# megapose6d/megapose6d

Hardware: NVIDIA H100
Metric: pose hypotheses/sec through render+coarse+5x refine (higher is better)
Workload: dtype f16

## Files before the change

include/mpx.h:

```cpp
#ifndef MPX_H_
#define MPX_H_

#include <stddef.h>
#include <stdint.h>

#ifdef __cplusplus
extern "C" {
#endif

#define MPX_ABI_VERSION 5

int mpx_abi_version(void);
int mpx_act_dtype(void);
const char* mpx_last_error(void);
long long mpx_launch_count(void);
int mpx_set_sm_limit(int n_sms);
int mpx_sm_count(void);
int mpx_profile_enable(int on);
int mpx_profile_summary(double* conv_ms, double* conv_flops, long long* conv_launches);

typedef struct mpx_meshdb mpx_meshdb;
int mpx_meshdb_create(int n_meshes, const float* h_verts, const float* h_normals,
                      const float* h_colors, const int64_t* h_vert_offsets, const int32_t* h_faces,
                      const int64_t* h_face_offsets, mpx_meshdb** out);
// ... 37 lines not shown
                          int c_in, void* d_x, int c_pad, int ch_per_view, const float* d_depth_norm_z,
                          void* d_workspace, size_t workspace_bytes, void* stream);

int mpx_pose_init_autodepth(const float* d_points, int n_pts, const int32_t* d_label_idx,
                            const float* d_bboxes, const float* d_K, const float* d_R, int n,
                            float* d_TCO, void* stream);

int mpx_normalize_T(const float* d_T_in, int n, float* d_T_out, void* stream);

int mpx_crop_geometry(const float* d_points, int n_pts, const int32_t* d_label_idx,
                      const float* d_TCO, const float* d_K, const float* d_tCR, int n, float lamb,
                      int im_h, int im_w, int out_h, int out_w, float* d_boxes_rend,
                      float* d_boxes_crop, float* d_K_crop, void* stream);

int mpx_multiview_cameras(const float* d_TCO, const float* d_tCR, int n, const float* h_offsets,
                          int n_extra, float* d_TCV_O, void* stream);

int mpx_pose_update(const float* d_TCO, const float* d_K_crop, const float* d_pose9,
                    const float* d_tCR, int n, float* d_TCO_out, void* stream);

int mpx_topk_per_group(const float* d_logits, int n_groups, int m, int k, int32_t* d_idx,
                       void* stream);

int mpx_image_to_nhwc4(const float* d_images_nchw, int b, int c, int h, int w, float* d_out_nhwc4,
                       void* stream);
int mpx_roi_align(const float* d_img_nhwc4, int b, int h, int w, const int32_t* d_im_idx,
                  const float* d_boxes, int n, int c, int out_h, int out_w, float* d_out,
                  void* stream);
int mpx_roi_align_fused(const float* d_img_nhwc4, int b, int h, int w, const int32_t* d_im_idx,
                        const float* d_boxes, int n, int c, int out_h, int out_w, void* d_x,
                        int c_pad, const float* d_depth_norm_z, int depth_norm_kind, void* stream);

size_t mpx_net_input_bytes(int n, int h, int w, int c_pad);

int mpx_conv2d(const void* d_x, int n, int h, int w, int c_in, const void* d_w,
                    const float* d_bias, int c_out, int r, int s, int stride, int pad_lo_h,
                    int pad_lo_w, int pad_hi_h, int pad_hi_w, int relu, const void* d_residual,
                    void* d_out, int block_n, int max_ctas, void* stream);

int mpx_conv2d_splitk(const void* d_x, int n, int h, int w, int c_in, const void* d_w,
                           const float* d_bias, int c_out, int r, int s, int stride, int pad_lo_h,
                           int pad_lo_w, int pad_hi_h, int pad_hi_w, int relu, const void* d_residual,
                           void* d_out, int block_n, int splits, void* stream);

#define MPX_CONV_NET_SPLITK 8
#define MPX_CONV_NO_PDL 512
#define MPX_CONV_SPLITK_CAP2 262144
#define MPX_CONV_SPLITK_CAP1 524288
#define MPX_CONV_NEVER_C64 4194304
#define MPX_CONV_FORCE_IM2COL 8388608
#define MPX_CONV_FORCE_C64 67108864
#define MPX_CONV_NEVER_PP 134217728
#define MPX_CONV_FORCE_PP 268435456
int mpx_conv_set_mode(int mode);

int mpx_maxpool3x3s2(const void* d_x, int n, int h, int w, int c, void* d_out, void* stream);

int mpx_avgpool_linear(const void* d_x, int n, int hw, int c, const float* d_w, const float* d_b,
                       int out_dim, float* d_out, void* stream);

typedef struct mpx_net mpx_net;
int mpx_net_create(int c_pad, int out_dim, const void* const* h_conv_w, const float* const* h_conv_b,
                   int n_convs, const float* d_head_w, const float* d_head_b, mpx_net** out);
int mpx_net_create_preact(int c_pad, int out_dim, const int32_t* h_layer_blocks, const void* const* h_conv_w,
                          const float* const* h_conv_b, int n_convs, const float* const* h_block_affine, int n_blocks,
                          const float* d_head_w, const float* d_head_b, mpx_net** out);
int mpx_net_destroy(mpx_net* net);
int mpx_net_set_graphs(int on);
size_t mpx_net_workspace_bytes(const mpx_net* net, int n, int h, int w);
int mpx_net_forward(const mpx_net* net, const void* d_x, int n, int h, int w, float* d_out,
                    void* d_workspace, size_t workspace_bytes, void* stream);

typedef struct mpx_fpn mpx_fpn;
int mpx_fpn_create(const void* const* h_conv_w, const float* const* h_conv_b, int n_convs, int n_anchors, mpx_fpn** out);
int mpx_fpn_destroy(mpx_fpn* fpn);
size_t mpx_fpn_workspace_bytes(int n, int h, int w);
int mpx_fpn_forward(const mpx_fpn* fpn, const float* d_images, int n, int h, int w, float* const* h_features,
                    float* const* h_objectness, float* const* h_deltas, void* d_workspace, size_t workspace_bytes,
                    void* stream);

int mpx_mask_paste(const float* d_logits, const int64_t* d_labels, const float* d_boxes, int n_masks, int n_classes,
                   int m, int n_images, const int32_t* h_counts, const int32_t* h_sizes, float* d_boxes_out,
                   float* const* h_masks, void* stream);

#define MPX_BOP_MAX_TAUS 16
int mpx_bop_vsd(int n_pairs, int h, int w, const uint16_t* d_depth_test, int n_img, const float* d_depth_scale,
                const double* d_K, const float* d_depth_est, int n_est, const float* d_depth_gt, int n_gt,
                const int32_t* d_est_idx, const int32_t* d_gt_idx, const int32_t* d_img_idx, const double* d_diameter,
                const double* h_taus, int n_taus, float delta, int64_t* d_counts, double* d_err, void* stream);

#define MPX_BOP_MSSD 0
#define MPX_BOP_MSPD 1
#define MPX_BOP_ADD 2
#define MPX_BOP_ADI 3
int mpx_bop_point_errors(int kind, int n_pairs, int n_models, const double* d_pts, const int64_t* d_pt_offsets,
                         long long n_pts_total, const double* d_syms, const int64_t* d_sym_offsets, long long n_syms_total,
                         const int32_t* d_model_idx, const double* d_pose_est, const double* d_pose_gt, const double* d_K,
                         double* d_err, int32_t* d_sym_argmin, void* stream);

int mpx_bop_gt_info(int n_gt, int h, int w, const uint16_t* d_depth_test, int n_img, const float* d_depth_scale,
                    const double* d_K, const float* d_depth_gt_large, const int32_t* d_img_idx, float delta,
                    int64_t* d_counts, int32_t* d_bbox, uint8_t* d_mask, uint8_t* d_mask_visib, void* stream);

#define MPX_TEASER_MAX_POINTS 1024
#define MPX_TEASER_MASK_SIMPLE 0
#define MPX_TEASER_MASK_THRESHOLD 1
// ... 28 lines not shown
```

megapose6d_b200/csrc/conv_wgmma.cu:

```cuda
#include <cuda.h>
#include <vector>
#include "mpx_common.cuh"

namespace mpx {

#ifdef MPX_ACT_BF16
#define kTmaActType CU_TENSOR_MAP_DATA_TYPE_BFLOAT16
#define MPX_WGMMA_AB "bf16.bf16"
#else
#define kTmaActType CU_TENSOR_MAP_DATA_TYPE_FLOAT16
#define MPX_WGMMA_AB "f16.f16"
#endif

__device__ __forceinline__ void mbar_init(uint64_t* bar, uint32_t count) {
  asm volatile("mbarrier.init.shared::cta.b64 [%0], %1;" ::"r"(smem_u32(bar)), "r"(count));
}
__device__ __forceinline__ void mbar_expect_tx(uint64_t* bar, uint32_t bytes) {
  asm volatile("mbarrier.arrive.expect_tx.shared::cta.b64 _, [%0], %1;" ::"r"(smem_u32(bar)), "r"(bytes) : "memory");
}
__device__ __forceinline__ void mbar_arrive(uint64_t* bar) {
  asm volatile("mbarrier.arrive.shared::cta.b64 _, [%0];" ::"r"(smem_u32(bar)) : "memory");
}
__device__ __forceinline__ bool mbar_try_wait(uint64_t* bar, uint32_t parity) {
  uint32_t ok;
  asm volatile(
      "{\n\t.reg .pred p;\n\t"
      "mbarrier.try_wait.parity.shared::cta.b64 p, [%1], %2;\n\t"
      "selp.u32 %0, 1, 0, p;\n\t}"
      : "=r"(ok)
      : "r"(smem_u32(bar)), "r"(parity)
      : "memory");
  return ok != 0;
}
__device__ __forceinline__ void mbar_wait(uint64_t* bar, uint32_t parity) {
  if (mbar_try_wait(bar, parity)) return;
  const long long t0 = clock64();
  while (!mbar_try_wait(bar, parity)) {
    if (clock64() - t0 > 8000000000LL) __trap();
  }
}

__device__ __forceinline__ void tma_load_2d(void* smem, const CUtensorMap* map, uint64_t* bar, int c0, int c1) {
  asm volatile(
      "cp.async.bulk.tensor.2d.shared::cluster.global.tile.mbarrier::complete_tx::bytes"
      " [%0], [%1, {%3, %4}], [%2];" ::"r"(smem_u32(smem)),
      "l"(map), "r"(smem_u32(bar)), "r"(c0), "r"(c1)
      : "memory");
}
__device__ __forceinline__ void tma_load_im2col_4d(void* smem, const CUtensorMap* map, uint64_t* bar, int c, int w, int h,
                                                   int n, uint16_t off_w, uint16_t off_h) {
  asm volatile(
      "cp.async.bulk.tensor.4d.shared::cluster.global.im2col.mbarrier::complete_tx::bytes"
      " [%0], [%1, {%3, %4, %5, %6}], [%2], {%7, %8};" ::"r"(smem_u32(smem)),
      "l"(map), "r"(smem_u32(bar)), "r"(c), "r"(w), "r"(h), "r"(n), "h"(off_w), "h"(off_h)
      : "memory");
}

__device__ __forceinline__ void wgmma_fence() { asm volatile("wgmma.fence.sync.aligned;" ::: "memory"); }
__device__ __forceinline__ void wgmma_commit() { asm volatile("wgmma.commit_group.sync.aligned;" ::: "memory"); }
template <int N>
__device__ __forceinline__ void wgmma_wait() {
  asm volatile("wgmma.wait_group.sync.aligned %0;" ::"n"(N) : "memory");
}

__device__ __forceinline__ void wgmma_m64n64k16(float (&d)[32], uint64_t desc_a, uint64_t desc_b, uint32_t accumulate) {
  asm volatile(
      "{\n\t.reg .pred p;\n\tsetp.ne.b32 p, %34, 0;\n\t"
      "wgmma.mma_async.sync.aligned.m64n64k16.f32." MPX_WGMMA_AB " "
      "{%0, %1, %2, %3, %4, %5, %6, %7, %8, %9, %10, %11, %12, %13, %14, %15, %16, %17, %18, %19, %20, %21, %22, %23, %24, %25, %26, %27, %28, %29, %30, %31}, %32, %33, p, 1, 1, 0, 0;\n\t}"
      : "+f"(d[0]), "+f"(d[1]), "+f"(d[2]), "+f"(d[3]), "+f"(d[4]), "+f"(d[5]), "+f"(d[6]), "+f"(d[7]), "+f"(d[8]), "+f"(d[9]), "+f"(d[10]), "+f"(d[11]), "+f"(d[12]), "+f"(d[13]), "+f"(d[14]), "+f"(d[15]), "+f"(d[16]), "+f"(d[17]), "+f"(d[18]), "+f"(d[19]), "+f"(d[20]), "+f"(d[21]), "+f"(d[22]), "+f"(d[23]), "+f"(d[24]), "+f"(d[25]), "+f"(d[26]), "+f"(d[27]), "+f"(d[28]), "+f"(d[29]), "+f"(d[30]), "+f"(d[31])
      : "l"(desc_a), "l"(desc_b), "r"(accumulate)
      : "memory");
}
__device__ __forceinline__ void wgmma_m64n128k16(float (&d)[64], uint64_t desc_a, uint64_t desc_b, uint32_t accumulate) {
  asm volatile(
      "{\n\t.reg .pred p;\n\tsetp.ne.b32 p, %66, 0;\n\t"
      "wgmma.mma_async.sync.aligned.m64n128k16.f32." MPX_WGMMA_AB " "
      "{%0, %1, %2, %3, %4, %5, %6, %7, %8, %9, %10, %11, %12, %13, %14, %15, %16, %17, %18, %19, %20, %21, %22, %23, %24, %25, %26, %27, %28, %29, %30, %31, %32, %33, %34, %35, %36, %37, %38, %39, %40, %41, %42, %43, %44, %45, %46, %47, %48, %49, %50, %51, %52, %53, %54, %55, %56, %57, %58, %59, %60, %61, %62, %63}, %64, %65, p, 1, 1, 0, 0;\n\t}"
      : "+f"(d[0]), "+f"(d[1]), "+f"(d[2]), "+f"(d[3]), "+f"(d[4]), "+f"(d[5]), "+f"(d[6]), "+f"(d[7]), "+f"(d[8]), "+f"(d[9]), "+f"(d[10]), "+f"(d[11]), "+f"(d[12]), "+f"(d[13]), "+f"(d[14]), "+f"(d[15]), "+f"(d[16]), "+f"(d[17]), "+f"(d[18]), "+f"(d[19]), "+f"(d[20]), "+f"(d[21]), "+f"(d[22]), "+f"(d[23]), "+f"(d[24]), "+f"(d[25]), "+f"(d[26]), "+f"(d[27]), "+f"(d[28]), "+f"(d[29]), "+f"(d[30]), "+f"(d[31]), "+f"(d[32]), "+f"(d[33]), "+f"(d[34]), "+f"(d[35]), "+f"(d[36]), "+f"(d[37]), "+f"(d[38]), "+f"(d[39]), "+f"(d[40]), "+f"(d[41]), "+f"(d[42]), "+f"(d[43]), "+f"(d[44]), "+f"(d[45]), "+f"(d[46]), "+f"(d[47]), "+f"(d[48]), "+f"(d[49]), "+f"(d[50]), "+f"(d[51]), "+f"(d[52]), "+f"(d[53]), "+f"(d[54]), "+f"(d[55]), "+f"(d[56]), "+f"(d[57]), "+f"(d[58]), "+f"(d[59]), "+f"(d[60]), "+f"(d[61]), "+f"(d[62]), "+f"(d[63])
      : "l"(desc_a), "l"(desc_b), "r"(accumulate)
      : "memory");
}
__device__ __forceinline__ void wgmma_m64n256k16(float (&d)[128], uint64_t desc_a, uint64_t desc_b, uint32_t accumulate) {
  asm volatile(
      "{\n\t.reg .pred p;\n\tsetp.ne.b32 p, %130, 0;\n\t"
      "wgmma.mma_async.sync.aligned.m64n256k16.f32." MPX_WGMMA_AB " "
      "{%0, %1, %2, %3, %4, %5, %6, %7, %8, %9, %10, %11, %12, %13, %14, %15, %16, %17, %18, %19, %20, %21, %22, %23, %24, %25, %26, %27, %28, %29, %30, %31, %32, %33, %34, %35, %36, %37, %38, %39, %40, %41, %42, %43, %44, %45, %46, %47, %48, %49, %50, %51, %52, %53, %54, %55, %56, %57, %58, %59, %60, %61, %62, %63, %64, %65, %66, %67, %68, %69, %70, %71, %72, %73, %74, %75, %76, %77, %78, %79, %80, %81, %82, %83, %84, %85, %86, %87, %88, %89, %90, %91, %92, %93, %94, %95, %96, %97, %98, %99, %100, %101, %102, %103, %104, %105, %106, %107, %108, %109, %110, %111, %112, %113, %114, %115, %116, %117, %118, %119, %120, %121, %122, %123, %124, %125, %126, %127}, %128, %129, p, 1, 1, 0, 0;\n\t}"
      : "+f"(d[0]), "+f"(d[1]), "+f"(d[2]), "+f"(d[3]), "+f"(d[4]), "+f"(d[5]), "+f"(d[6]), "+f"(d[7]), "+f"(d[8]), "+f"(d[9]), "+f"(d[10]), "+f"(d[11]), "+f"(d[12]), "+f"(d[13]), "+f"(d[14]), "+f"(d[15]), "+f"(d[16]), "+f"(d[17]), "+f"(d[18]), "+f"(d[19]), "+f"(d[20]), "+f"(d[21]), "+f"(d[22]), "+f"(d[23]), "+f"(d[24]), "+f"(d[25]), "+f"(d[26]), "+f"(d[27]), "+f"(d[28]), "+f"(d[29]), "+f"(d[30]), "+f"(d[31]), "+f"(d[32]), "+f"(d[33]), "+f"(d[34]), "+f"(d[35]), "+f"(d[36]), "+f"(d[37]), "+f"(d[38]), "+f"(d[39]), "+f"(d[40]), "+f"(d[41]), "+f"(d[42]), "+f"(d[43]), "+f"(d[44]), "+f"(d[45]), "+f"(d[46]), "+f"(d[47]), "+f"(d[48]), "+f"(d[49]), "+f"(d[50]), "+f"(d[51]), "+f"(d[52]), "+f"(d[53]), "+f"(d[54]), "+f"(d[55]), "+f"(d[56]), "+f"(d[57]), "+f"(d[58]), "+f"(d[59]), "+f"(d[60]), "+f"(d[61]), "+f"(d[62]), "+f"(d[63]), "+f"(d[64]), "+f"(d[65]), "+f"(d[66]), "+f"(d[67]), "+f"(d[68]), "+f"(d[69]), "+f"(d[70]), "+f"(d[71]), "+f"(d[72]), "+f"(d[73]), "+f"(d[74]), "+f"(d[75]), "+f"(d[76]), "+f"(d[77]), "+f"(d[78]), "+f"(d[79]), "+f"(d[80]), "+f"(d[81]), "+f"(d[82]), "+f"(d[83]), "+f"(d[84]), "+f"(d[85]), "+f"(d[86]), "+f"(d[87]), "+f"(d[88]), "+f"(d[89]), "+f"(d[90]), "+f"(d[91]), "+f"(d[92]), "+f"(d[93]), "+f"(d[94]), "+f"(d[95]), "+f"(d[96]), "+f"(d[97]), "+f"(d[98]), "+f"(d[99]), "+f"(d[100]), "+f"(d[101]), "+f"(d[102]), "+f"(d[103]), "+f"(d[104]), "+f"(d[105]), "+f"(d[106]), "+f"(d[107]), "+f"(d[108]), "+f"(d[109]), "+f"(d[110]), "+f"(d[111]), "+f"(d[112]), "+f"(d[113]), "+f"(d[114]), "+f"(d[115]), "+f"(d[116]), "+f"(d[117]), "+f"(d[118]), "+f"(d[119]), "+f"(d[120]), "+f"(d[121]), "+f"(d[122]), "+f"(d[123]), "+f"(d[124]), "+f"(d[125]), "+f"(d[126]), "+f"(d[127])
      : "l"(desc_a), "l"(desc_b), "r"(accumulate)
      : "memory");
}
__device__ __forceinline__ void wgmma_m64n160k16(float (&d)[80], uint64_t desc_a, uint64_t desc_b, uint32_t accumulate) {
  asm volatile(
      "{\n\t.reg .pred p;\n\tsetp.ne.b32 p, %82, 0;\n\t"
      "wgmma.mma_async.sync.aligned.m64n160k16.f32." MPX_WGMMA_AB " "
      "{%0, %1, %2, %3, %4, %5, %6, %7, %8, %9, %10, %11, %12, %13, %14, %15, %16, %17, %18, %19, %20, %21, %22, %23, %24, %25, %26, %27, %28, %29, %30, %31, %32, %33, %34, %35, %36, %37, %38, %39, %40, %41, %42, %43, %44, %45, %46, %47, %48, %49, %50, %51, %52, %53, %54, %55, %56, %57, %58, %59, %60, %61, %62, %63, %64, %65, %66, %67, %68, %69, %70, %71, %72, %73, %74, %75, %76, %77, %78, %79}, %80, %81, p, 1, 1, 0, 0;\n\t}"
      : "+f"(d[0]), "+f"(d[1]), "+f"(d[2]), "+f"(d[3]), "+f"(d[4]), "+f"(d[5]), "+f"(d[6]), "+f"(d[7]), "+f"(d[8]), "+f"(d[9]), "+f"(d[10]), "+f"(d[11]), "+f"(d[12]), "+f"(d[13]), "+f"(d[14]), "+f"(d[15]), "+f"(d[16]), "+f"(d[17]), "+f"(d[18]), "+f"(d[19]), "+f"(d[20]), "+f"(d[21]), "+f"(d[22]), "+f"(d[23]), "+f"(d[24]), "+f"(d[25]), "+f"(d[26]), "+f"(d[27]), "+f"(d[28]), "+f"(d[29]), "+f"(d[30]), "+f"(d[31]), "+f"(d[32]), "+f"(d[33]), "+f"(d[34]), "+f"(d[35]), "+f"(d[36]), "+f"(d[37]), "+f"(d[38]), "+f"(d[39]), "+f"(d[40]), "+f"(d[41]), "+f"(d[42]), "+f"(d[43]), "+f"(d[44]), "+f"(d[45]), "+f"(d[46]), "+f"(d[47]), "+f"(d[48]), "+f"(d[49]), "+f"(d[50]), "+f"(d[51]), "+f"(d[52]), "+f"(d[53]), "+f"(d[54]), "+f"(d[55]), "+f"(d[56]), "+f"(d[57]), "+f"(d[58]), "+f"(d[59]), "+f"(d[60]), "+f"(d[61]), "+f"(d[62]), "+f"(d[63]), "+f"(d[64]), "+f"(d[65]), "+f"(d[66]), "+f"(d[67]), "+f"(d[68]), "+f"(d[69]), "+f"(d[70]), "+f"(d[71]), "+f"(d[72]), "+f"(d[73]), "+f"(d[74]), "+f"(d[75]), "+f"(d[76]), "+f"(d[77]), "+f"(d[78]), "+f"(d[79])
      : "l"(desc_a), "l"(desc_b), "r"(accumulate)
      : "memory");
}
template <int BLOCK_N>
__device__ __forceinline__ void wgmma_tile(float (&d)[BLOCK_N / 2], uint64_t da, uint64_t db, uint32_t accumulate) {
  if constexpr (BLOCK_N == 64) wgmma_m64n64k16(d, da, db, accumulate);
  else if constexpr (BLOCK_N == 128) wgmma_m64n128k16(d, da, db, accumulate);
  else if constexpr (BLOCK_N == 160) wgmma_m64n160k16(d, da, db, accumulate);
  else wgmma_m64n256k16(d, da, db, accumulate);
}

__device__ __forceinline__ uint64_t make_sw128_desc(uint32_t smem_addr) {
// ... 48 lines not shown
}
int conv_profile_summary(double* total_ms, double* total_flops, long long* launches) {
  MPX_CHECK_CUDA(cudaDeviceSynchronize());
  double ms = 0, fl = 0;
  for (size_t i = 0; i < g_slots_used; ++i) {
    float t = 0.f;
    MPX_CHECK_CUDA(cudaEventElapsedTime(&t, g_slots[i].e0, g_slots[i].e1));
    ms += t;
    fl += g_slots[i].flops;
  }
  *total_ms = ms;
  *total_flops = fl;
  *launches = static_cast<long long>(g_slots_used);
  g_slots_used = 0;
  return MPX_OK;
}

static int g_conv_mode = MPX_CONV_NET_SPLITK;
int conv_get_mode() { return g_conv_mode; }
void conv_set_mode(int mode) { g_conv_mode = mode; }

struct ConvParams {
  int M_total;
  int P, Q;
  int C_out;
  int S;
  int stride;
  int pad_h, pad_w;
  int cblocks;
  int num_k_blocks;
  int m_tiles, n_tiles;
  int relu;
  const float* bias;
  const act_t* residual;
  act_t* out;
  int splits;
};

constexpr int kBlockM = 128;
constexpr int kBlockK = 64;
constexpr int kATileBytes = kBlockM * kBlockK * 2;
constexpr int kThreads = 384;

template <int BLOCK_N>
struct ConvCfg {
  static constexpr int kBTileBytes = BLOCK_N * kBlockK * 2;
  static constexpr int kStageBytes = kATileBytes + kBTileBytes;
  static constexpr int kStages = (BLOCK_N == 256) ? 4 : (BLOCK_N == 128 ? 6 : 8);
  static constexpr int kSmemBytes =
      kStages * kStageBytes + 1024  + 256  + 2048 ;
  static int smem_bytes(int c_out) { return c_out <= 512 ? kSmemBytes : kSmemBytes - 2048 + 4 * c_out; }
  static constexpr int kParkPitch = BLOCK_N * 4 + 16;
  static_assert(kBlockM * kParkPitch <= kStages * kStageBytes, "split-K tile does not fit the pipeline stages");
};

template <int NCOLS>
__device__ __forceinline__ void splitk_reduce_slice(uint32_t tile_smem, int splits, int rank, long long m0, int M_total,
                                                    int C_out, int n0, act_t* __restrict__ out,
                                                    const act_t* __restrict__ residual, const float* bias_s, int relu,
                                                    int tid, int nthreads) {
  constexpr int kVecPerRow = NCOLS / 4;
  const int rows_per = kBlockM / splits;
  for (int u = tid; u < rows_per * kVecPerRow; u += nthreads) {
    const int r = rank * rows_per + u / kVecPerRow;
    const int c = (u % kVecPerRow) * 4;
    const long long m = m0 + r;
    if (m >= M_total) continue;
    const uint32_t local = tile_smem + static_cast<uint32_t>(r * ConvCfg<NCOLS>::kParkPitch + c * 4);
    float4 part[8];
#pragma unroll
    for (int sp = 0; sp < 8; ++sp) {
      if (sp < splits) {
        uint32_t remote;
        asm volatile("mapa.shared::cluster.u32 %0, %1, %2;" : "=r"(remote) : "r"(local), "r"(sp));
        asm volatile("ld.shared::cluster.v4.f32 {%0, %1, %2, %3}, [%4];"
                     : "=f"(part[sp].x), "=f"(part[sp].y), "=f"(part[sp].z), "=f"(part[sp].w)
                     : "r"(remote)
                     : "memory");
      }
    }
    float4 a = part[0];
#pragma unroll
    for (int sp = 1; sp < 8; ++sp)
      if (sp < splits) { a.x += part[sp].x; a.y += part[sp].y; a.z += part[sp].z; a.w += part[sp].w; }
    const float4 b4 = *reinterpret_cast<const float4*>(bias_s + c);
    float f[4] = {a.x + b4.x, a.y + b4.y, a.z + b4.z, a.w + b4.w};
    const size_t off = static_cast<size_t>(m) * C_out + n0 + c;
    if (residual != nullptr) {
      const uint2 rr = __ldg(reinterpret_cast<const uint2*>(residual + off));
      const float2 t0 = unpack_act2(rr.x), t1 = unpack_act2(rr.y);
      f[0] += t0.x; f[1] += t0.y; f[2] += t1.x; f[3] += t1.y;
    }
    if (relu) {
#pragma unroll
      for (int j = 0; j < 4; ++j) f[j] = fmaxf(f[j], 0.f);
    }
    uint2 o;
    o.x = pack_act2(f[0], f[1]);
    o.y = pack_act2(f[2], f[3]);
    *reinterpret_cast<uint2*>(out + off) = o;
  }
}

template <int BLOCK_N>
__global__ void __launch_bounds__(kThreads, 1)
conv_wgmma_kernel(const __grid_constant__ CUtensorMap map_a, const __grid_constant__ CUtensorMap map_b,
                  const ConvParams p) {
  using Cfg = ConvCfg<BLOCK_N>;
  constexpr int kStages = Cfg::kStages;
  extern __shared__ uint8_t smem_raw[];
  uint8_t* smem = reinterpret_cast<uint8_t*>((reinterpret_cast<uintptr_t>(smem_raw) + 1023) &
                                             ~static_cast<uintptr_t>(1023));
  uint8_t* smem_a = smem;
  uint8_t* smem_b = smem + kStages * kATileBytes;
  uint64_t* bars = reinterpret_cast<uint64_t*>(smem + kStages * Cfg::kStageBytes);
  uint64_t* full_bar = bars;
  uint64_t* empty_bar = bars + kStages;
  float* bias_s = reinterpret_cast<float*>(bars + 32);

  const int wg = __shfl_sync(0xffffffffu, threadIdx.x >> 7, 0);
  const int total_tiles = p.m_tiles * p.n_tiles * p.splits;
  for (int i = threadIdx.x; i < p.C_out; i += blockDim.x) bias_s[i] = p.bias[i];

  if (threadIdx.x == 0) {
    asm volatile("prefetch.tensormap [%0];" ::"l"(&map_a) : "memory");
    asm volatile("prefetch.tensormap [%0];" ::"l"(&map_b) : "memory");
    for (int i = 0; i < kStages; ++i) {
      mbar_init(&full_bar[i], 1);
      mbar_init(&empty_bar[i], 8);
    }
    asm volatile("fence.mbarrier_init.release.cluster;" ::: "memory");
  }
  pdl_trigger();
  __syncthreads();
  pdl_wait();

  if (wg == 0) {
    if (threadIdx.x == 0) {
      int stage = 0;
      uint32_t phase = 0;
      const int pq = p.P * p.Q;
      for (int item = blockIdx.x; item < total_tiles; item += gridDim.x) {
        const int tile = item / p.splits;
        const int split = item - tile * p.splits;
        const int kb_begin = split * p.num_k_blocks / p.splits;
        const int kb_end = (split + 1) * p.num_k_blocks / p.splits;
        const int m_tile = tile / p.n_tiles;
        const int n_tile = tile - m_tile * p.n_tiles;
        const int m0 = m_tile * kBlockM;
        const int img = m0 / pq;
        const int rem = m0 - img * pq;
        const int p0 = rem / p.Q;
        const int q0 = rem - p0 * p.Q;
        const int base_w = q0 * p.stride - p.pad_w;
        const int base_h = p0 * p.stride - p.pad_h;
        int tap = kb_begin / p.cblocks, cb = kb_begin - tap * p.cblocks;
        for (int kb = kb_begin; kb < kb_end; ++kb) {
          mbar_wait(&empty_bar[stage], phase ^ 1u);
          mbar_expect_tx(&full_bar[stage], Cfg::kStageBytes);
          const int r = tap / p.S;
          const int s = tap - r * p.S;
          tma_load_im2col_4d(smem_a + stage * kATileBytes, &map_a, &full_bar[stage], cb * kBlockK, base_w, base_h, img,
                             static_cast<uint16_t>(s), static_cast<uint16_t>(r));
          tma_load_2d(smem_b + stage * Cfg::kBTileBytes, &map_b, &full_bar[stage], kb * kBlockK, n_tile * BLOCK_N);
          if (++cb == p.cblocks) {
            cb = 0;
            ++tap;
          }
          if (++stage == kStages) {
            stage = 0;
            phase ^= 1u;
          }
        }
      }
    }
  } else {
    const int half = wg - 1;
    const int t = threadIdx.x & 127;
    const int lane = threadIdx.x & 31;
    const int row_lo = half * 64 + (t >> 5) * 16 + (lane >> 2);
    const int col = 2 * (lane & 3);
    int stage = 0;
    uint32_t phase = 0;
    for (int item = blockIdx.x; item < total_tiles; item += gridDim.x) {
      const int tile = item / p.splits;
      const int split = item - tile * p.splits;
      const int kb_begin = split * p.num_k_blocks / p.splits;
      const int kb_end = (split + 1) * p.num_k_blocks / p.splits;
      const int m_tile = tile / p.n_tiles;
      const int n_tile = tile - m_tile * p.n_tiles;
      float acc[BLOCK_N / 2];
#pragma unroll
      for (int i = 0; i < BLOCK_N / 2; ++i) acc[i] = 0.f;
      int prev_stage = -1;
      for (int kb = kb_begin; kb < kb_end; ++kb) {
        mbar_wait(&full_bar[stage], phase);
        const uint64_t da = make_sw128_desc(smem_u32(smem_a + stage * kATileBytes + half * 64 * 128));
        const uint64_t db = make_sw128_desc(smem_u32(smem_b + stage * Cfg::kBTileBytes));
        wgmma_fence();
#pragma unroll
        for (int k = 0; k < kBlockK / 16; ++k)
          wgmma_tile<BLOCK_N>(acc, da + static_cast<uint64_t>(2 * k), db + static_cast<uint64_t>(2 * k), 1u);
        wgmma_commit();
        wgmma_wait<1>();
        if (prev_stage >= 0) {
          __syncwarp();
          if (lane == 0) mbar_arrive(&empty_bar[prev_stage]);
        }
        prev_stage = stage;
        if (++stage == kStages) {
          stage = 0;
          phase ^= 1u;
        }
      }
      wgmma_wait<0>();
      if (prev_stage >= 0) {
        __syncwarp();
        if (lane == 0) mbar_arrive(&empty_bar[prev_stage]);
      }
      const long long m0 = static_cast<long long>(m_tile) * kBlockM;
      const int n0 = n_tile * BLOCK_N;
      if (p.splits > 1) {
        consumers_sync();
        const uint32_t park = smem_u32(smem);
#pragma unroll
        for (int h = 0; h < 2; ++h) {
          const uint32_t rbase = park + static_cast<uint32_t>((row_lo + 8 * h) * Cfg::kParkPitch + col * 4);
#pragma unroll
          for (int j = 0; j < BLOCK_N / 8; ++j)
            asm volatile("st.shared.v2.f32 [%0], {%1, %2};" ::"r"(rbase + static_cast<uint32_t>(32 * j)),
                         "f"(acc[4 * j + 2 * h]), "f"(acc[4 * j + 2 * h + 1])
                         : "memory");
        }
        continue;
      }
#pragma unroll
      for (int h = 0; h < 2; ++h) {
        const long long m = m0 + row_lo + 8 * h;
        const bool valid = m < p.M_total;
        const size_t off = static_cast<size_t>(valid ? m : 0) * p.C_out + n0 + col;
        if (!valid) continue;
        const act_t* res_row = p.residual ? p.residual + off : nullptr;
        uint32_t packed[BLOCK_N / 8];
#pragma unroll
        for (int j = 0; j < BLOCK_N / 8; ++j) {
          const float2 b = *reinterpret_cast<const float2*>(bias_s + n0 + 8 * j + col);
          float f0 = acc[4 * j + 2 * h] + b.x;
          float f1 = acc[4 * j + 2 * h + 1] + b.y;
          if (res_row) {
            const float2 r = unpack_act2(__ldg(reinterpret_cast<const uint32_t*>(res_row + 8 * j)));
            f0 += r.x;
            f1 += r.y;
          }
          if (p.relu) {
            f0 = fmaxf(f0, 0.f);
            f1 = fmaxf(f1, 0.f);
          }
          packed[j] = pack_act2(f0, f1);
        }
#pragma unroll
        for (int j = 0; j < BLOCK_N / 8; ++j) *reinterpret_cast<uint32_t*>(p.out + off + 8 * j) = packed[j];
      }
    }
  }

  __syncthreads();
  if (p.splits > 1) {
    cluster_sync_all();
    const int item = blockIdx.x;
    const int tile = item / p.splits;
    const int m_tile = tile / p.n_tiles;
    const int n_tile = tile - m_tile * p.n_tiles;
    const int n0 = n_tile * BLOCK_N;
    splitk_reduce_slice<BLOCK_N>(smem_u32(smem), p.splits, static_cast<int>(cluster_ctarank()),
                                 static_cast<long long>(m_tile) * kBlockM, p.M_total, p.C_out, n0, p.out, p.residual,
                                 bias_s + n0, p.relu, threadIdx.x, blockDim.x);
    cluster_sync_all();
  }
}

constexpr int kC64Pixels = 256;
constexpr int kC64Stages = 4;
constexpr int kC64ActBytes = kC64Pixels * kBlockK * 2;
constexpr int kC64WBytes = 64 * kBlockK * 2;
constexpr int kC64StageBytes = kC64ActBytes + kC64WBytes;
constexpr int kC64StagingBytes = kC64Pixels * 64 * 2;
constexpr int kC64BandSlots = 3;
constexpr int kC64BandWStages = 8;
static_assert(kC64BandSlots * kC64ActBytes + kC64BandWStages * kC64WBytes == kC64Stages * kC64StageBytes,
              "conv64: the band producer's ring layout is the im2col producer's");
constexpr int kC64SmemBytes = 227 * 1024;
constexpr int kC64BufferBytes = kC64SmemBytes - 1024  - 256  - 256 ;
static_assert(kC64Stages * kC64StageBytes + 2 * kC64StagingBytes <= kC64BufferBytes, "conv64: shared memory budget");

struct Conv64Params {
  int M_total, P, Q, S, stride, pad_h, pad_w, cblocks, num_k_blocks, m_tiles;
  int band_w, band_rows, tiles_per_img;
  int band_slots, slot_bytes, w_resident, w_off, staging_off, staging_bytes;
  int relu;
  int has_residual;
  const float* bias;
};

__device__ __forceinline__ void tma_store_2d(const CUtensorMap* map, const void* smem, int c0, int c1) {
  asm volatile("cp.async.bulk.tensor.2d.global.shared::cta.bulk_group [%0, {%2, %3}], [%1];" ::"l"(map),
               "r"(smem_u32(smem)), "r"(c0), "r"(c1)
               : "memory");
}
__device__ __forceinline__ void tma_load_4d(void* smem, const CUtensorMap* map, uint64_t* bar, int c0, int c1, int c2,
                                            int c3) {
  asm volatile(
      "cp.async.bulk.tensor.4d.shared::cluster.global.tile.mbarrier::complete_tx::bytes"
      " [%0], [%1, {%3, %4, %5, %6}], [%2];" ::"r"(smem_u32(smem)),
      "l"(map), "r"(smem_u32(bar)), "r"(c0), "r"(c1), "r"(c2), "r"(c3)
      : "memory");
}
__device__ __forceinline__ void tma_store_4d(const CUtensorMap* map, const void* smem, int c0, int c1, int c2, int c3) {
  asm volatile("cp.async.bulk.tensor.4d.global.shared::cta.bulk_group [%0, {%2, %3, %4, %5}], [%1];" ::"l"(map),
               "r"(smem_u32(smem)), "r"(c0), "r"(c1), "r"(c2), "r"(c3)
               : "memory");
}
__device__ __forceinline__ void bulk_commit() { asm volatile("cp.async.bulk.commit_group;" ::: "memory"); }
__device__ __forceinline__ void bulk_wait_read_all() { asm volatile("cp.async.bulk.wait_group.read 0;" ::: "memory"); }
__device__ __forceinline__ void bulk_wait_all() { asm volatile("cp.async.bulk.wait_group 0;" ::: "memory"); }
__device__ __forceinline__ void fence_proxy_async_smem() { asm volatile("fence.proxy.async.shared::cta;" ::: "memory"); }
__device__ __forceinline__ void warpgroup_sync(int cw) { asm volatile("bar.sync %0, 128;" ::"r"(2 + cw) : "memory"); }
__device__ __forceinline__ void mainloop_turn_wait(int cw) { asm volatile("bar.sync %0, 256;" ::"r"(4 + cw) : "memory"); }
__device__ __forceinline__ void mainloop_turn_pass(int cw) { asm volatile("bar.arrive %0, 256;" ::"r"(5 - cw) : "memory"); }

__host__ __device__ __forceinline__ uint32_t stem_live_steps(int kb, int cblocks, int S) {
  const int tap = kb / cblocks, cb = kb - tap * cblocks;
  const int r = tap / S, s = tap - r * S;
  uint32_t live = 0;
  for (int k = 0; k < 4; ++k) {
    const int slice = (4 * cb + k) / cblocks;
    const int ky = 2 * r + (slice >> 1) - 1, kx = 2 * s + (slice & 1) - 1;
    if (ky >= 0 && ky <= 6 && kx >= 0 && kx <= 6) live |= 1u << k;
  }
  return live;
}

template <int N>
__device__ __forceinline__ void wgmma_kblock(uint32_t live, float (&acc)[N / 2], uint64_t da, uint64_t db) {
  wgmma_fence();
#pragma unroll
  for (int k = 0; k < kBlockK / 16; ++k)
    if (live & (1u << k)) wgmma_tile<N>(acc, da + static_cast<uint64_t>(2 * k), db + static_cast<uint64_t>(2 * k), 1u);
  wgmma_commit();
}

template <int kStemCblocks, int kBandN>
__global__ void __launch_bounds__(kThreads, 1)
conv64_wgmma_kernel(const __grid_constant__ CUtensorMap map_x, const __grid_constant__ CUtensorMap map_w,
                    const __grid_constant__ CUtensorMap map_res, const __grid_constant__ CUtensorMap map_out,
                    const Conv64Params p) {
  constexpr bool kBand = kBandN > 0;
  constexpr int kN = kBand ? kBandN : kC64Pixels;
  constexpr int kStages = kBand ? kC64BandWStages : kC64Stages;
  extern __shared__ uint8_t smem_raw[];
  uint8_t* smem = reinterpret_cast<uint8_t*>((reinterpret_cast<uintptr_t>(smem_raw) + 1023) &
                                             ~static_cast<uintptr_t>(1023));
  uint8_t* smem_x = smem;
  uint8_t* smem_w = smem + (kBand ? p.w_off : kC64Stages * kC64ActBytes);
  uint8_t* staging = smem + (kBand ? p.staging_off : kC64Stages * kC64StageBytes);
  const int staging_bytes = kBand ? p.staging_bytes : kC64StagingBytes;
  const int slot_bytes = kBand ? p.slot_bytes : kC64ActBytes;
  const bool w_resident = kBand && p.w_resident;
  uint64_t* bars = reinterpret_cast<uint64_t*>(smem + kC64BufferBytes);
  uint64_t* full_bar = bars;
  uint64_t* empty_bar = bars + 8;
  uint64_t* res_bar = bars + 16;
  uint64_t* band_full = bars + 18;
  uint64_t* band_empty = bars + 21;
  uint64_t* w_bar = bars + 24;
  float* bias_s = reinterpret_cast<float*>(bars + 32);

  const int wg = __shfl_sync(0xffffffffu, threadIdx.x >> 7, 0);
  const int nk = p.num_k_blocks;
  for (int i = threadIdx.x; i < 64; i += blockDim.x) bias_s[i] = p.bias[i];
// ... 427 lines not shown
              const float2 r = unpack_act2(rr);
              f0 += r.x;
              f1 += r.y;
            }
            if (p.relu) {
              f0 = fmaxf(f0, 0.f);
              f1 = fmaxf(f1, 0.f);
            }
            asm volatile("st.shared.b32 [%0], %1;" ::"r"(addr), "r"(pack_act2(f0, f1)) : "memory");
          }
        }
      }
      fence_proxy_async_smem();
      warpgroup_sync(cw);
      if (t == 0) {
        tma_store_2d(&map_out, stage_buf, n0, m0);
        tma_store_2d(&map_out, stage_buf + kPPStagingBytes / 2, n0 + 64, m0);
        bulk_commit();
      }
    }
    if (t == 0) bulk_wait_all();
  }
}

typedef CUresult (*PFN_encodeTiled)(CUtensorMap*, CUtensorMapDataType, cuuint32_t, void*,
                                    const cuuint64_t*, const cuuint64_t*, const cuuint32_t*,
                                    const cuuint32_t*, CUtensorMapInterleave, CUtensorMapSwizzle,
                                    CUtensorMapL2promotion, CUtensorMapFloatOOBfill);
typedef CUresult (*PFN_encodeIm2col)(CUtensorMap*, CUtensorMapDataType, cuuint32_t, void*,
                                     const cuuint64_t*, const cuuint64_t*, const int*, const int*,
                                     cuuint32_t, cuuint32_t, const cuuint32_t*, CUtensorMapInterleave,
                                     CUtensorMapSwizzle, CUtensorMapL2promotion,
                                     CUtensorMapFloatOOBfill);

static PFN_encodeTiled g_encode_tiled = nullptr;
static PFN_encodeIm2col g_encode_im2col = nullptr;

static int load_driver_entry_points() {
  if (g_encode_tiled && g_encode_im2col) return MPX_OK;
  cudaDriverEntryPointQueryResult q;
  void* f = nullptr;
  MPX_CHECK_CUDA(cudaGetDriverEntryPoint("cuTensorMapEncodeTiled", &f, cudaEnableDefault, &q));
  MPX_REQUIRE(f != nullptr && q == cudaDriverEntryPointSuccess,
              "cuTensorMapEncodeTiled not available from the driver");
  g_encode_tiled = reinterpret_cast<PFN_encodeTiled>(f);
  f = nullptr;
  MPX_CHECK_CUDA(cudaGetDriverEntryPoint("cuTensorMapEncodeIm2col", &f, cudaEnableDefault, &q));
  MPX_REQUIRE(f != nullptr && q == cudaDriverEntryPointSuccess,
              "cuTensorMapEncodeIm2col not available from the driver");
  g_encode_im2col = reinterpret_cast<PFN_encodeIm2col>(f);
  return MPX_OK;
}

template <int BLOCK_N>
static int launch_conv(const CUtensorMap& ma, const CUtensorMap& mb, const ConvParams& p, cudaStream_t stream,
                       int max_ctas) {
  using Cfg = ConvCfg<BLOCK_N>;
  const int smem = Cfg::smem_bytes(p.C_out);
  static int attr_bytes = 0;
  if (smem > attr_bytes) {
    MPX_CHECK_CUDA(cudaFuncSetAttribute(conv_wgmma_kernel<BLOCK_N>, cudaFuncAttributeMaxDynamicSharedMemorySize, smem));
    attr_bytes = smem;
  }
  int grid = p.m_tiles * p.n_tiles * p.splits;
  const int cap = max_ctas > 0 ? max_ctas : sm_count();
  ProfileSlot* slot = profile_begin(stream);
  if (p.splits == 1 && grid > cap) grid = cap;
  MPX_CHECK_CUDA(launch_pdl(conv_wgmma_kernel<BLOCK_N>, dim3(grid), dim3(kThreads), smem, stream, p.splits,
                            ma, mb, p));
  MPX_CHECK_CUDA(cudaGetLastError());
  ++g_launches;
  profile_end(slot, stream, 2.0 * p.M_total * p.C_out * p.num_k_blocks * kBlockK);
  return MPX_OK;
}

int conv_out_dim(int in, int pad_lo, int pad_hi, int k, int stride) {
  return (in + pad_lo + pad_hi - k) / stride + 1;
}

static int encode_im2col_map(CUtensorMap* map, const ConvDesc& d, const void* x) {
  cuuint64_t dims[4] = {static_cast<cuuint64_t>(d.C_in), static_cast<cuuint64_t>(d.W),
                        static_cast<cuuint64_t>(d.H), static_cast<cuuint64_t>(d.n_img)};
  cuuint64_t strides[3] = {static_cast<cuuint64_t>(d.C_in) * 2,
                           static_cast<cuuint64_t>(d.W) * d.C_in * 2,
                           static_cast<cuuint64_t>(d.H) * d.W * d.C_in * 2};
  int lower[2] = {-d.pad_lo_w, -d.pad_lo_h};
  int upper[2] = {d.pad_hi_w - (d.S - 1), d.pad_hi_h - (d.R - 1)};
  cuuint32_t estr[4] = {1, static_cast<cuuint32_t>(d.stride), static_cast<cuuint32_t>(d.stride), 1};
  CUresult r = g_encode_im2col(map, kTmaActType, 4, const_cast<void*>(x),
                               dims, strides, lower, upper, kBlockK,
                               kBlockM, estr, CU_TENSOR_MAP_INTERLEAVE_NONE,
                               CU_TENSOR_MAP_SWIZZLE_128B, CU_TENSOR_MAP_L2_PROMOTION_L2_128B,
                               CU_TENSOR_MAP_FLOAT_OOB_FILL_NONE);
  MPX_REQUIRE(r == CUDA_SUCCESS, "cuTensorMapEncodeIm2col failed (%d)", static_cast<int>(r));
  int drv = 0;
  cudaDriverGetVersion(&drv);
  const size_t bytes = static_cast<size_t>(d.n_img) * d.H * d.W * d.C_in * 2;
  if (drv <= 13010 && bytes < 131072) {
    reinterpret_cast<uint64_t*>(map)[1] &= ~(1ull << 21);
  }
  return MPX_OK;
}

static int encode_2d_map(CUtensorMap* map, const void* ptr, cuuint64_t cols, cuuint64_t rows, int box_cols, int box_rows,
                         CUtensorMapL2promotion promo) {
  cuuint64_t dims[2] = {cols, rows};
  cuuint64_t strides[1] = {cols * 2};
  cuuint32_t box[2] = {static_cast<cuuint32_t>(box_cols), static_cast<cuuint32_t>(box_rows)};
  cuuint32_t estr[2] = {1, 1};
  CUresult r = g_encode_tiled(map, kTmaActType, 2, const_cast<void*>(ptr), dims, strides, box, estr,
                              CU_TENSOR_MAP_INTERLEAVE_NONE, CU_TENSOR_MAP_SWIZZLE_128B, promo,
                              CU_TENSOR_MAP_FLOAT_OOB_FILL_NONE);
  MPX_REQUIRE(r == CUDA_SUCCESS, "cuTensorMapEncodeTiled failed (%d)", static_cast<int>(r));
  return MPX_OK;
}

static int encode_nhwc_map(CUtensorMap* map, const void* ptr, int n, int H, int W, int C, int box_w, int box_h) {
  cuuint64_t dims[4] = {static_cast<cuuint64_t>(C), static_cast<cuuint64_t>(W), static_cast<cuuint64_t>(H),
                        static_cast<cuuint64_t>(n)};
  cuuint64_t strides[3] = {static_cast<cuuint64_t>(C) * 2, static_cast<cuuint64_t>(W) * C * 2,
                           static_cast<cuuint64_t>(H) * W * C * 2};
  cuuint32_t box[4] = {static_cast<cuuint32_t>(kBlockK), static_cast<cuuint32_t>(box_w), static_cast<cuuint32_t>(box_h),
// ... 198 lines not shown
      return conv64_forward(d, x, w, bias, residual, out, static_cast<int>(M_total), P, Q, cap, stream);
  }

  const long long m_tiles = (M_total + kBlockM - 1) / kBlockM;
  if (d.C_out % 128 == 0 && d.C_out <= 512 && block_n_override == 0 && splitk <= 0 && aligned &&
      (g_conv_mode & MPX_CONV_NEVER_PP) == 0 &&
      ((g_conv_mode & MPX_CONV_FORCE_PP) != 0 || (d.C_out == 128 && m_tiles >= 2LL * cap))) {
    const int nkb = d.R * d.S * (d.C_in / kBlockK);
    if (!(splitk < 0 && m_tiles * (d.C_out / block_n) * 2 <= cap && nkb >= 8))
      return convpp_forward(d, x, w, bias, residual, out, static_cast<int>(M_total), P, Q, cap, stream);
  }

  CUtensorMap map_a, map_b;
  rc = encode_im2col_map(&map_a, d, x);
  if (rc != MPX_OK) return rc;
  rc = encode_2d_map(&map_b, w, static_cast<cuuint64_t>(d.R) * d.S * d.C_in, d.C_out, kBlockK, block_n,
                     CU_TENSOR_MAP_L2_PROMOTION_L2_256B);
  if (rc != MPX_OK) return rc;

  ConvParams p{};
  p.M_total = static_cast<int>(M_total);
  p.P = P;
  p.Q = Q;
  p.C_out = d.C_out;
  p.S = d.S;
  p.stride = d.stride;
  p.pad_h = d.pad_lo_h;
  p.pad_w = d.pad_lo_w;
  p.cblocks = d.C_in / kBlockK;
  p.num_k_blocks = d.R * d.S * p.cblocks;
  p.m_tiles = static_cast<int>((M_total + kBlockM - 1) / kBlockM);
  p.n_tiles = d.C_out / block_n;
  p.relu = d.relu;
  p.bias = bias;
  p.residual = reinterpret_cast<const act_t*>(residual);
  p.out = reinterpret_cast<act_t*>(out);
  p.splits = 1;
  if (splitk != 0) {
    const int tiles = p.m_tiles * p.n_tiles;
    const int sms = max_ctas > 0 ? max_ctas : sm_count();
    int want = splitk > 0 ? splitk : 1;
    if (splitk < 0 && tiles * 2 <= sms && p.num_k_blocks >= 8) {
      want = p.num_k_blocks / 4;
      if (want > sms / tiles) want = sms / tiles;
    }
    const int cap = (splitk < 0 && (g_conv_mode & MPX_CONV_SPLITK_CAP1))
                        ? 1
                        : ((splitk < 0 && (g_conv_mode & MPX_CONV_SPLITK_CAP2)) ? 2 : 8);
    int splits = 1;
    while (splits * 2 <= want && splits * 2 <= cap && splits * 2 <= p.num_k_blocks) splits *= 2;
    p.splits = splits;
  }

  switch (block_n) {
    case 64:
      return launch_conv<64>(map_a, map_b, p, stream, max_ctas);
    case 128:
      return launch_conv<128>(map_a, map_b, p, stream, max_ctas);
    default:
      return launch_conv<256>(map_a, map_b, p, stream, max_ctas);
  }
}

}
```

Measured before the change: 30050.

## Stage conv epilogue through shared memory with TMA residual loads and stores

For 128x256 non-split-K conv tiles, the epilogue now packs results into swizzled shared-memory staging buffers and writes them with TMA bulk tensor stores instead of scattered per-thread global stores. Residual tiles are prefetched by TMA during the mainloop, half into a staging buffer and half through a pipeline stage slot, so the residual add reads shared memory. Register budgets are rebalanced with setmaxnreg between producer and consumer warpgroups. This adds shared-memory pressure, extra barriers and complexity in stage/phase accounting, which risks correctness or stalls.

```diff
diff --git a/include/mpx.h b/include/mpx.h
--- a/include/mpx.h
+++ b/include/mpx.h
@@ -113,6 +113,7 @@
 #define MPX_CONV_FORCE_C64 67108864
 #define MPX_CONV_NEVER_PP 134217728
 #define MPX_CONV_FORCE_PP 268435456
+#define MPX_CONV_DIRECT_EPILOGUE 536870912
 int mpx_conv_set_mode(int mode);
 
 int mpx_maxpool3x3s2(const void* d_x, int n, int h, int w, int c, void* d_out, void* stream);
diff --git a/megapose6d_b200/csrc/conv_wgmma.cu b/megapose6d_b200/csrc/conv_wgmma.cu
--- a/megapose6d_b200/csrc/conv_wgmma.cu
+++ b/megapose6d_b200/csrc/conv_wgmma.cu
@@ -55,6 +55,17 @@
       "l"(map), "r"(smem_u32(bar)), "r"(c), "r"(w), "r"(h), "r"(n), "h"(off_w), "h"(off_h)
       : "memory");
 }
+
+__device__ __forceinline__ void tma_store_2d(const CUtensorMap* map, const void* smem, int c0, int c1) {
+  asm volatile("cp.async.bulk.tensor.2d.global.shared::cta.bulk_group [%0, {%2, %3}], [%1];" ::"l"(map),
+               "r"(smem_u32(smem)), "r"(c0), "r"(c1)
+               : "memory");
+}
+__device__ __forceinline__ void bulk_commit() { asm volatile("cp.async.bulk.commit_group;" ::: "memory"); }
+__device__ __forceinline__ void bulk_wait_read_all() { asm volatile("cp.async.bulk.wait_group.read 0;" ::: "memory"); }
+__device__ __forceinline__ void bulk_wait_all() { asm volatile("cp.async.bulk.wait_group 0;" ::: "memory"); }
+__device__ __forceinline__ void fence_proxy_async_smem() { asm volatile("fence.proxy.async.shared::cta;" ::: "memory"); }
+__device__ __forceinline__ void warpgroup_sync(int cw) { asm volatile("bar.sync %0, 128;" ::"r"(2 + cw) : "memory"); }
 
 __device__ __forceinline__ void wgmma_fence() { asm volatile("wgmma.fence.sync.aligned;" ::: "memory"); }
 __device__ __forceinline__ void wgmma_commit() { asm volatile("wgmma.commit_group.sync.aligned;" ::: "memory"); }
@@ -209,7 +220,11 @@
   static int smem_bytes(int c_out) { return c_out <= 512 ? kSmemBytes : kSmemBytes - 2048 + 4 * c_out; }
   static constexpr int kParkPitch = BLOCK_N * 4 + 16;
   static_assert(kBlockM * kParkPitch <= kStages * kStageBytes, "split-K tile does not fit the pipeline stages");
+  static constexpr int kBoxBytes = 64 * 64 * 2;
+  static constexpr int kStagingBytes = 2 * kBoxBytes;
+  static constexpr int kStagedSmemBytes = kStages * kStageBytes + 2 * kStagingBytes + 1024  + 256;
 };
+static_assert(ConvCfg<256>::kStagedSmemBytes <= 232448, "staged epilogue: shared memory budget");
 
 template <int NCOLS>
 __device__ __forceinline__ void splitk_reduce_slice(uint32_t tile_smem, int splits, int rank, long long m0, int M_total,
@@ -259,29 +274,40 @@
   }
 }
 
-template <int BLOCK_N>
+template <int BLOCK_N, bool kStaged>
 __global__ void __launch_bounds__(kThreads, 1)
 conv_wgmma_kernel(const __grid_constant__ CUtensorMap map_a, const __grid_constant__ CUtensorMap map_b,
+                  const __grid_constant__ CUtensorMap map_res, const __grid_constant__ CUtensorMap map_out,
                   const ConvParams p) {
   using Cfg = ConvCfg<BLOCK_N>;
   constexpr int kStages = Cfg::kStages;
+  static_assert(!kStaged || BLOCK_N == 256, "the staged epilogue serves 128 x 256 tiles");
   extern __shared__ uint8_t smem_raw[];
   uint8_t* smem = reinterpret_cast<uint8_t*>((reinterpret_cast<uintptr_t>(smem_raw) + 1023) &
                                              ~static_cast<uintptr_t>(1023));
   uint8_t* smem_a = smem;
   uint8_t* smem_b = smem + kStages * kATileBytes;
-  uint64_t* bars = reinterpret_cast<uint64_t*>(smem + kStages * Cfg::kStageBytes);
+  uint8_t* staging = smem + kStages * Cfg::kStageBytes;
+  uint64_t* bars = reinterpret_cast<uint64_t*>(staging + (kStaged ? 2 * Cfg::kStagingBytes : 0));
   uint64_t* full_bar = bars;
   uint64_t* empty_bar = bars + kStages;
+  uint64_t* res_bar = bars + 16;
   float* bias_s = reinterpret_cast<float*>(bars + 32);
 
   const int wg = __shfl_sync(0xffffffffu, threadIdx.x >> 7, 0);
   const int total_tiles = p.m_tiles * p.n_tiles * p.splits;
-  for (int i = threadIdx.x; i < p.C_out; i += blockDim.x) bias_s[i] = p.bias[i];
+  if constexpr (!kStaged)
+    for (int i = threadIdx.x; i < p.C_out; i += blockDim.x) bias_s[i] = p.bias[i];
 
   if (threadIdx.x == 0) {
     asm volatile("prefetch.tensormap [%0];" ::"l"(&map_a) : "memory");
     asm volatile("prefetch.tensormap [%0];" ::"l"(&map_b) : "memory");
+    if constexpr (kStaged) {
+      asm volatile("prefetch.tensormap [%0];" ::"l"(&map_out) : "memory");
+      if (p.residual) asm volatile("prefetch.tensormap [%0];" ::"l"(&map_res) : "memory");
+      mbar_init(&res_bar[0], 1);
+      mbar_init(&res_bar[1], 1);
+    }
     for (int i = 0; i < kStages; ++i) {
       mbar_init(&full_bar[i], 1);
       mbar_init(&empty_bar[i], 8);
@@ -293,6 +319,7 @@
   pdl_wait();
 
   if (wg == 0) {
+    if constexpr (kStaged) asm volatile("setmaxnreg.dec.sync.aligned.u32 40;");
     if (threadIdx.x == 0) {
       int stage = 0;
       uint32_t phase = 0;
@@ -329,14 +356,29 @@
             phase ^= 1u;
           }
         }
+        if (kStaged && p.residual) {
+          mbar_wait(&empty_bar[stage], phase ^ 1u);
+          mbar_expect_tx(&full_bar[stage], 4 * Cfg::kBoxBytes);
+          uint8_t* dst = smem_b + stage * Cfg::kBTileBytes;
+          for (int b = 0; b < 4; ++b)
+            tma_load_2d(dst + b * Cfg::kBoxBytes, &map_res, &full_bar[stage], n_tile * BLOCK_N + 128 + 64 * (b & 1),
+                        m0 + 64 * (b >> 1));
+          if (++stage == kStages) {
+            stage = 0;
+            phase ^= 1u;
+          }
+        }
       }
     }
   } else {
+    if constexpr (kStaged) asm volatile("setmaxnreg.inc.sync.aligned.u32 232;");
     const int half = wg - 1;
     const int t = threadIdx.x & 127;
     const int lane = threadIdx.x & 31;
     const int row_lo = half * 64 + (t >> 5) * 16 + (lane >> 2);
     const int col = 2 * (lane & 3);
+    uint8_t* stage_buf = staging + half * Cfg::kStagingBytes;
+    uint32_t res_phase = 0;
     int stage = 0;
     uint32_t phase = 0;
     for (int item = blockIdx.x; item < total_tiles; item += gridDim.x) {
@@ -346,6 +388,7 @@
       const int kb_end = (split + 1) * p.num_k_blocks / p.splits;
       const int m_tile = tile / p.n_tiles;
       const int n_tile = tile - m_tile * p.n_tiles;
+      const int res_kb = kb_end - kb_begin > 2 ? kb_begin + 2 : kb_end - 1;
       float acc[BLOCK_N / 2];
 #pragma unroll
       for (int i = 0; i < BLOCK_N / 2; ++i) acc[i] = 0.f;
@@ -359,6 +402,15 @@
         for (int k = 0; k < kBlockK / 16; ++k)
           wgmma_tile<BLOCK_N>(acc, da + static_cast<uint64_t>(2 * k), db + static_cast<uint64_t>(2 * k), 1u);
         wgmma_commit();
+        if constexpr (kStaged) {
+          if (p.residual && t == 0 && kb == res_kb) {
+            bulk_wait_read_all();
+            mbar_expect_tx(&res_bar[half], Cfg::kStagingBytes);
+            tma_load_2d(stage_buf, &map_res, &res_bar[half], n_tile * BLOCK_N, m_tile * kBlockM + 64 * half);
+            tma_load_2d(stage_buf + Cfg::kBoxBytes, &map_res, &res_bar[half], n_tile * BLOCK_N + 64,
+                        m_tile * kBlockM + 64 * half);
+          }
+        }
         wgmma_wait<1>();
         if (prev_stage >= 0) {
           __syncwarp();
@@ -377,6 +429,77 @@
       }
       const long long m0 = static_cast<long long>(m_tile) * kBlockM;
       const int n0 = n_tile * BLOCK_N;
+      if constexpr (kStaged) {
+        const uint32_t sbase = smem_u32(stage_buf);
+        const int wrow = row_lo - 64 * half;
+        const int gm = m_tile * kBlockM + 64 * half;
+#pragma unroll
+        for (int pass = 0; pass < 2; ++pass) {
+          const uint32_t rsrc = pass == 0 ? sbase : smem_u32(smem_b + stage * Cfg::kBTileBytes + half * 2 * Cfg::kBoxBytes);
+          if (p.residual) {
+            if (pass == 0) {
+              mbar_wait(&res_bar[half], res_phase);
+              res_phase ^= 1u;
+            } else {
+              mbar_wait(&full_bar[stage], phase);
+            }
+          }
+          uint32_t packed[2][16];
+#pragma unroll
+          for (int h = 0; h < 2; ++h) {
+            const int row = wrow + 8 * h;
+            const uint32_t roff = static_cast<uint32_t>(row * 128 + col * 2);
+#pragma unroll
+            for (int jj = 0; jj < 16; ++jj) {
+              const int j = 16 * pass + jj;
+              float f0 = acc[4 * j + 2 * h] + __ldg(p.bias + n0 + 8 * j + col);
+              float f1 = acc[4 * j + 2 * h + 1] + __ldg(p.bias + n0 + 8 * j + col + 1);
+              if (p.residual) {
+                const uint32_t off = roff + static_cast<uint32_t>((jj >> 3) * Cfg::kBoxBytes + (((jj & 7) ^ (row & 7)) << 4));
+                uint32_t rr;
+                asm volatile("ld.shared.b32 %0, [%1];" : "=r"(rr) : "r"(rsrc + off) : "memory");
+                const float2 r = unpack_act2(rr);
+                f0 += r.x;
+                f1 += r.y;
+              }
+              if (p.relu) {
+                f0 = fmaxf(f0, 0.f);
+                f1 = fmaxf(f1, 0.f);
+              }
+              packed[h][jj] = pack_act2(f0, f1);
+            }
+          }
+          if (pass == 1 && p.residual) {
+            __syncwarp();
+            if (lane == 0) mbar_arrive(&empty_bar[stage]);
+            if (++stage == kStages) {
+              stage = 0;
+              phase ^= 1u;
+            }
+          }
+          if (t == 0) bulk_wait_read_all();
+          warpgroup_sync(half);
+#pragma unroll
+          for (int h = 0; h < 2; ++h) {
+            const int row = wrow + 8 * h;
+            const uint32_t roff = static_cast<uint32_t>(row * 128 + col * 2);
+#pragma unroll
+            for (int jj = 0; jj < 16; ++jj) {
+              const uint32_t addr =
+                  sbase + roff + static_cast<uint32_t>((jj >> 3) * Cfg::kBoxBytes + (((jj & 7) ^ (row & 7)) << 4));
+              asm volatile("st.shared.b32 [%0], %1;" ::"r"(addr), "r"(packed[h][jj]) : "memory");
+            }
+          }
+          fence_proxy_async_smem();
+          warpgroup_sync(half);
+          if (t == 0) {
+            tma_store_2d(&map_out, stage_buf, n0 + 128 * pass, gm);
+            tma_store_2d(&map_out, stage_buf + Cfg::kBoxBytes, n0 + 128 * pass + 64, gm);
+            bulk_commit();
+          }
+        }
+        continue;
+      }
       if (p.splits > 1) {
         consumers_sync();
         const uint32_t park = smem_u32(smem);
@@ -419,10 +542,12 @@
         for (int j = 0; j < BLOCK_N / 8; ++j) *reinterpret_cast<uint32_t*>(p.out + off + 8 * j) = packed[j];
       }
     }
+    if constexpr (kStaged)
+      if (t == 0) bulk_wait_all();
   }
 
   __syncthreads();
-  if (p.splits > 1) {
+  if (!kStaged && p.splits > 1) {
     cluster_sync_all();
     const int item = blockIdx.x;
     const int tile = item / p.splits;
@@ -459,11 +584,6 @@
   const float* bias;
 };
 
-__device__ __forceinline__ void tma_store_2d(const CUtensorMap* map, const void* smem, int c0, int c1) {
-  asm volatile("cp.async.bulk.tensor.2d.global.shared::cta.bulk_group [%0, {%2, %3}], [%1];" ::"l"(map),
-               "r"(smem_u32(smem)), "r"(c0), "r"(c1)
-               : "memory");
-}
 __device__ __forceinline__ void tma_load_4d(void* smem, const CUtensorMap* map, uint64_t* bar, int c0, int c1, int c2,
                                             int c3) {
   asm volatile(
@@ -477,11 +597,6 @@
                "r"(smem_u32(smem)), "r"(c0), "r"(c1), "r"(c2), "r"(c3)
                : "memory");
 }
-__device__ __forceinline__ void bulk_commit() { asm volatile("cp.async.bulk.commit_group;" ::: "memory"); }
-__device__ __forceinline__ void bulk_wait_read_all() { asm volatile("cp.async.bulk.wait_group.read 0;" ::: "memory"); }
-__device__ __forceinline__ void bulk_wait_all() { asm volatile("cp.async.bulk.wait_group 0;" ::: "memory"); }
-__device__ __forceinline__ void fence_proxy_async_smem() { asm volatile("fence.proxy.async.shared::cta;" ::: "memory"); }
-__device__ __forceinline__ void warpgroup_sync(int cw) { asm volatile("bar.sync %0, 128;" ::"r"(2 + cw) : "memory"); }
 __device__ __forceinline__ void mainloop_turn_wait(int cw) { asm volatile("bar.sync %0, 256;" ::"r"(4 + cw) : "memory"); }
 __device__ __forceinline__ void mainloop_turn_pass(int cw) { asm volatile("bar.arrive %0, 256;" ::"r"(5 - cw) : "memory"); }
 
@@ -1015,22 +1130,23 @@
   return MPX_OK;
 }
 
-template <int BLOCK_N>
-static int launch_conv(const CUtensorMap& ma, const CUtensorMap& mb, const ConvParams& p, cudaStream_t stream,
-                       int max_ctas) {
+template <int BLOCK_N, bool kStaged>
+static int launch_conv(const CUtensorMap& ma, const CUtensorMap& mb, const CUtensorMap& mres, const CUtensorMap& mout,
+                       const ConvParams& p, cudaStream_t stream, int max_ctas) {
   using Cfg = ConvCfg<BLOCK_N>;
-  const int smem = Cfg::smem_bytes(p.C_out);
+  const int smem = kStaged ? Cfg::kStagedSmemBytes : Cfg::smem_bytes(p.C_out);
   static int attr_bytes = 0;
   if (smem > attr_bytes) {
-    MPX_CHECK_CUDA(cudaFuncSetAttribute(conv_wgmma_kernel<BLOCK_N>, cudaFuncAttributeMaxDynamicSharedMemorySize, smem));
+    MPX_CHECK_CUDA(cudaFuncSetAttribute(conv_wgmma_kernel<BLOCK_N, kStaged>, cudaFuncAttributeMaxDynamicSharedMemorySize,
+                                        smem));
     attr_bytes = smem;
   }
   int grid = p.m_tiles * p.n_tiles * p.splits;
   const int cap = max_ctas > 0 ? max_ctas : sm_count();
   ProfileSlot* slot = profile_begin(stream);
   if (p.splits == 1 && grid > cap) grid = cap;
-  MPX_CHECK_CUDA(launch_pdl(conv_wgmma_kernel<BLOCK_N>, dim3(grid), dim3(kThreads), smem, stream, p.splits,
-                            ma, mb, p));
+  MPX_CHECK_CUDA(launch_pdl(conv_wgmma_kernel<BLOCK_N, kStaged>, dim3(grid), dim3(kThreads), smem, stream, p.splits,
+                            ma, mb, mres, mout, p));
   MPX_CHECK_CUDA(cudaGetLastError());
   ++g_launches;
   profile_end(slot, stream, 2.0 * p.M_total * p.C_out * p.num_k_blocks * kBlockK);
@@ -1335,14 +1451,25 @@
     p.splits = splits;
   }
 
+  if (block_n == 256 && p.splits == 1 && aligned && (g_conv_mode & MPX_CONV_DIRECT_EPILOGUE) == 0) {
+    CUtensorMap map_res, map_out;
+    rc = encode_2d_map(&map_out, out, d.C_out, M_total, 64, 64, CU_TENSOR_MAP_L2_PROMOTION_L2_128B);
+    if (rc != MPX_OK) return rc;
+    map_res = map_out;
+    if (residual != nullptr) {
+      rc = encode_2d_map(&map_res, residual, d.C_out, M_total, 64, 64, CU_TENSOR_MAP_L2_PROMOTION_L2_128B);
+      if (rc != MPX_OK) return rc;
+    }
+    return launch_conv<256, true>(map_a, map_b, map_res, map_out, p, stream, max_ctas);
+  }
   switch (block_n) {
     case 64:
-      return launch_conv<64>(map_a, map_b, p, stream, max_ctas);
+      return launch_conv<64, false>(map_a, map_b, map_a, map_a, p, stream, max_ctas);
     case 128:
-      return launch_conv<128>(map_a, map_b, p, stream, max_ctas);
+      return launch_conv<128, false>(map_a, map_b, map_a, map_a, p, stream, max_ctas);
     default:
-      return launch_conv<256>(map_a, map_b, p, stream, max_ctas);
-  }
-}
-
-}
+      return launch_conv<256, false>(map_a, map_b, map_a, map_a, p, stream, max_ctas);
+  }
+}
+
+}
```

Measured after the change: 30720 (median of 6 runs). +2.2%, better.
